# TissueImageAnalytics/cerberus

Measured on AMD Instinct MI355X. Metric: Mpx/sec WSI tiled inference (all heads), higher is better.
Workload: dtype f32

## Files before the change

### cerberus_amd/csrc/cerb_api.hip

```cpp
#include "cerb_net.h"

static thread_local std::string g_err;
int cerb_set_error(const std::string& m) {
    g_err = m;
    return 1;
}
extern "C" int cerb_version(void) { return 4; }
extern "C" const char* cerb_last_error(void) { return g_err.c_str(); }
std::atomic<long long> g_devbuf_bytes{0};
extern "C" size_t cerb_device_bytes_held(void) { const long long v = g_devbuf_bytes.load(); return v > 0 ? (size_t)v : 0; }
thread_local hipStream_t g_call_stream = nullptr;

static int alloc_dev(cerb_net* net, size_t bytes, void** out) {
    if (net->reusing) {
        if (net->reuse_cursor >= net->n_finalize_allocs || net->dev_alloc_bytes[net->reuse_cursor] != bytes)
            return fail("reload: the tensors do not have the shapes the handle was finalized with");
        *out = net->dev_allocs[net->reuse_cursor++];
        return 0;
    }
    void* d = nullptr;
    HIP_OK(hipMalloc(&d, bytes));
    net->dev_allocs.push_back(d);
    net->dev_alloc_bytes.push_back(bytes);
    *out = d;
// ... 718 lines not shown
            cur = net->x[li + 1].p;
            inpl = planes;
            continue;
        }
        for (int b = 0; b < kLayers[li]; ++b) {
            const std::string p = "backbone.layer" + std::to_string(li + 1) + "." + std::to_string(b);
            const int stride = (b == 0 && li > 0) ? 2 : 1;
            const int hin = (b == 0) ? Hi : hh, win = (b == 0) ? Wi : ww;
            float* t1 = net->ta.p;
            float* outb = ((kLayers[li] - 1 - b) % 2 == 0) ? net->x[li + 1].p : net->tb.p;
            const float* idt = cur;
            if (run_conv(net, p + ".conv1", {.in = cur, .out = t1, .N = N, .H = hin, .W = win, .relu = 1}, st)) return 1;
            if (stride != 1 || inpl != planes) {
                if (run_conv(net, p + ".downsample", {.in = cur, .out = net->pool.p, .N = N, .H = hin, .W = win}, st)) return 1;
                idt = net->pool.p;
            }
            if (run_conv(net, p + ".conv2", {.in = t1, .resid = idt, .out = outb, .N = N, .H = hh, .W = ww, .relu = 1}, st)) return 1;
            cur = outb;
            inpl = planes;
        }
    }
    if (run_conv(net, "conv_map", {.in = net->x[4].p, .out = net->cm.p, .N = N, .H = hs[4], .W = ws[4]}, st)) return 1;

    const long long tile_stride = io->tile_stride ? io->tile_stride : (long long)out_h * out_w;
    const long long row_stride = io->row_stride ? io->row_stride : out_w;
    if (net->pc_idx >= 0) {
        const bool want = io->out && io->out[net->pc_idx];
        const bool wantl = io->logits && io->logits[net->pc_idx];
        if (want || wantl) {
            PatchClassParams pp;
            memset(&pp, 0, sizeof(pp));
            pp.x4 = net->x[4].p; pp.bn1_s = net->pc_bn1s; pp.bn1_b = net->pc_bn1b; pp.w1t = net->pc_w1t; pp.b1 = net->pc_b1;
            pp.w2t = net->pc_w2t; pp.b2 = net->pc_b2;
            pp.N = N; pp.Hf = hs[4]; pp.Wf = ws[4]; pp.out_ch = net->dec[net->pc_idx].out_ch;
            pp.out_h = out_h; pp.out_w = out_w;
            pp.logits = wantl ? io->logits[net->pc_idx] : nullptr;
            pp.out = want ? (float*)io->out[net->pc_idx] : nullptr;
            pp.tile_off = io->tile_off; pp.tile_stride = tile_stride; pp.row_stride = row_stride;
            PROF("patch_class", "patch_class", 2.0 * N * (512.0 * 256 + 256.0 * pp.out_ch), HIP_OK(cerb_launch_patch_class(pp, st)));
        }
    }
    if (D) {
        const float* skips[4] = {net->x[3].p, net->x[2].p, net->x[1].p, net->x0.p};
        const float* prev = net->cm.p;
        long long prev_gs = 0;
        const int oc[4] = {128, 64, 64, 64};
        int roi_out[4][4], roi_mid[4][4], roi_sum[4][4];
        const bool any_logits = [&] {
            if (!io->logits) return false;
            for (size_t k = 0; k < net->dec.size(); ++k)
                if (io->logits[k]) return true;
            return false;
        }();
        const bool use_roi = net->crop_roi && (net->conv_algo == 1 || net->conv_algo >= 5) && !any_logits && (out_h < H || out_w < W);
        if (use_roi) {
            int y0 = (int)((H - out_h) * 0.5), x0 = (int)((W - out_w) * 0.5), y1 = y0 + out_h, x1 = x0 + out_w;
            for (int u = 3; u >= 0; --u) {
                const int hh = hs[3 - u], ww = ws[3 - u];
                auto widen = [&](int* r, const int* in, int d) {
                    r[0] = std::max(0, (in[0] - d) & ~3); r[1] = std::min(hh, (in[1] + d + 3) & ~3);
                    r[2] = std::max(0, (in[2] - d) & ~3); r[3] = std::min(ww, (in[3] + d + 3) & ~3);
                };
                const int win[4] = {y0, y1, x0, x1};
                widen(roi_out[u], win, 0);
                widen(roi_mid[u], roi_out[u], 1);
                widen(roi_sum[u], roi_mid[u], 1);
                y0 = std::max(0, roi_sum[u][0] / 2 - 1); y1 = std::min(hh / 2, (roi_sum[u][1] - 1) / 2 + 2);
                x0 = std::max(0, roi_sum[u][2] / 2 - 1); x1 = std::min(ww / 2, (roi_sum[u][3] - 1) / 2 + 2);
            }
        }
        bool feat_planar = false, prev_planar = false;
        for (int u = 0; u < 4; ++u) {
            const int hh = hs[3 - u], ww = ws[3 - u];
            const std::string n0 = "dec." + std::to_string(u) + ".0", n1 = "dec." + std::to_string(u) + ".1";
            const int cmid = net->conv[n0].cout;
            const int cin0 = net->conv[n0].cin;
            const int* r_sum = use_roi ? roi_sum[u] : nullptr;
            const int* r_mid = use_roi ? roi_mid[u] : nullptr;
            const int* r_out = use_roi ? roi_out[u] : nullptr;
            if (level_is_planar[u]) {
                PlanarBuf &bs = net->dec_sum[u], &bm = net->dec_mid[u];
                const int cout1 = net->conv[n1].cout;
                PlanarBuf& bo = cout1 == cin0 ? bs : net->dec_out[u];
                if (bs.ensure((int)D, N, hh, ww, cin0, st) || bm.ensure((int)D, N, hh, ww, cmid, st) || (&bo != &bs && bo.ensure((int)D, N, hh, ww, cout1, st)))
                    return fail_alloc();
                PROF(n0 + ".up", kPlanarEntryFamily[u], 0.0, HIP_OK(cerb_launch_upsample2_add_planar(skips[u], prev, bs.b.p, (int)D, N, hh, ww, cin0, prev_gs, bs.gs(), r_sum, prev_planar ? 1 : 0, st)));
                if (run_conv(net, n0, {.in = bs.b.p, .out = bm.b.p, .N = N, .H = hh, .W = ww, .relu = 1, .in_gs = bs.gs(), .roi = r_mid, .planar_out_gs = bm.gs(), .site = u}, st)) return 1;
                if (run_conv(net, n1, {.in = bm.b.p, .out = bo.b.p, .N = N, .H = hh, .W = ww, .relu = 1, .in_gs = bm.gs(), .roi = r_out, .planar_out_gs = bo.gs(), .site = u}, st)) return 1;
                if (u == 3) feat_planar = true;
                prev = bo.b.p;
                prev_gs = bo.gs();
                prev_planar = true;
                continue;
            }
            if (prev_planar) return fail("internal: a tile-planar decoder level feeds an NHWC one");
            if (net->conv_algo && net->conv[n0].wino) {
                PROF(n0 + ".up", "upsample2_add", 0.0, HIP_OK(cerb_launch_upsample2_add(skips[u], prev, net->dsum.p, (int)D, N, hh, ww, cin0, prev_gs, r_sum, st)));
                if (run_conv(net, n0, {.in = net->dsum.p, .out = net->dmid.p, .N = N, .H = hh, .W = ww, .relu = 1, .in_gs = (long long)N * hh * ww * cin0, .roi = r_mid}, st)) return 1;
            } else if (run_conv(net, n0, {.in = skips[u], .prev = prev, .out = net->dmid.p, .N = N, .H = hh, .W = ww, .relu = 1, .mode = 1, .prev_gs = prev_gs}, st)) return 1;
            if (run_conv(net, n1, {.in = net->dmid.p, .out = net->dout[u].p, .N = N, .H = hh, .W = ww, .relu = 1, .in_gs = (long long)N * hh * ww * cmid, .roi = r_out}, st)) return 1;
            prev = net->dout[u].p;
            prev_gs = (long long)N * hh * ww * oc[u];
        }
        HeadParams hps[8];
        int n_hp = 0;
        double head_flops = 0.0;
        for (size_t k = 0; k < net->dense_idx.size(); ++k) {
            const int di = net->dense_idx[k];
            const size_t tk = (size_t)net->trunk_of[k];
            const DecoderCfg& d = net->dec[di];
            const bool want = io->out && io->out[di];
            const bool wantl = io->logits && io->logits[di];
            if (!(want || wantl)) continue;
            HeadParams hp;
            memset(&hp, 0, sizeof(hp));
            hp.feat = feat_planar ? net->dec_sum[3].b.p + tk * net->dec_sum[3].gs() : net->dout[3].p + tk * (size_t)N * H * W * 64;
            hp.feat_planar = feat_planar ? 1 : 0;
            hp.pl_byp = cerb_planar_blocks(H);
            hp.pl_bxp = cerb_planar_blocks(W);
            hp.w1p = net->head_w1[k]; hp.b1 = net->head_b1[k]; hp.w2p = net->head_w2[k]; hp.b2 = net->head_b2[k]; hp.w2q = net->head_w2q[k];
            hp.N = N; hp.H = H; hp.W = W; hp.out_ch = d.out_ch; hp.kind = d.kind;
            hp.crop_y0 = (int)((H - out_h) * 0.5); hp.crop_x0 = (int)((W - out_w) * 0.5);
            hp.out_h = want ? out_h : 0; hp.out_w = want ? out_w : 0;
            hp.roi = use_roi ? 1 : 0;
            hp.logits = wantl ? io->logits[di] : nullptr;
            hp.absmax_bits = io->logit_absmax ? io->logit_absmax + di : nullptr;
            if (want) {
                if (d.kind == 0) hp.out_inst = (float*)io->out[di];
                else if (io->type_is_u8) hp.out_type_u8 = (unsigned char*)io->out[di];
                else hp.out_type_i64 = (long long*)io->out[di];
            }
            hp.tile_off = io->tile_off; hp.tile_stride = tile_stride; hp.row_stride = row_stride;
            const double head_px = hp.roi ? (double)out_h * (((hp.crop_x0 + out_w + 15) / 16 - hp.crop_x0 / 16) * 16.0) : (double)H * W;
            const double fl = 2.0 * N * head_px * (64.0 * 96 + 96.0 * d.out_ch);
            if (net->head_algo == 0) {
                PROF("head." + d.name, "head", fl, HIP_OK(cerb_launch_head(hp, st)));
            } else {
                if (n_hp == 8) {
                    PROF("heads", "head_group", head_flops, HIP_OK(cerb_launch_head_group(hps, n_hp, st, net->head_algo == 1 ? 1 : 0)));
                    n_hp = 0;
                    head_flops = 0.0;
                }
                hps[n_hp++] = hp;
                head_flops += fl;
            }
        }
        if (n_hp > 0) {
            PROF("heads", "head_group", head_flops, HIP_OK(cerb_launch_head_group(hps, n_hp, st, net->head_algo == 1 ? 1 : 0)));
        }
    }
    if (io->feats) {
        const float* src[6] = {net->x0.p, net->x[1].p, net->x[2].p, net->x[3].p, net->cm.p, net->x[4].p};
        const size_t nb[6] = {(size_t)N * H * W * 64, (size_t)N * hs[1] * ws[1] * 64, (size_t)N * hs[2] * ws[2] * 128,
                              (size_t)N * hs[3] * ws[3] * 256, (size_t)N * hs[4] * ws[4] * 256, (size_t)N * hs[4] * ws[4] * 512};
        for (int i = 0; i < 6; ++i)
            if (io->feats[i]) HIP_OK(hipMemcpyAsync(io->feats[i], src[i], nb[i] * 4, hipMemcpyDeviceToDevice, st));
    }
    return 0;
}

extern "C" int cerb_net_begin_reload(cerb_net* net) {
    if (!net) return fail("cerb_net_begin_reload: null handle");
    HIP_OK(hipDeviceSynchronize());
    while (net->dev_allocs.size() > net->n_finalize_allocs) {
        (void)hipFree(net->dev_allocs.back());
        net->dev_allocs.pop_back();
        net->dev_alloc_bytes.pop_back();
    }
    net->reusing = true;
    net->reuse_cursor = 0;
    net->param_slots.clear();
    net->conv.clear();
    net->bn.clear();
    net->raw.clear();
    net->grads.clear();
    net->head_w1.clear(); net->head_b1.clear(); net->head_w2.clear(); net->head_b2.clear(); net->head_w2q.clear();
    net->head_rw1.clear(); net->head_rb1.clear(); net->head_rw2.clear(); net->head_rb2.clear();
    net->host.clear();
    net->finalized = false;
    return 0;
}
// ... 176 lines not shown
```

### cerberus_amd/csrc/net_kernels.hip

```cpp
#include "cerb_common.h"

struct StemParams {
    const unsigned char* tiles;
    const float* tiles_f32;
    const float* wpack;
    const float* bias;
    float* out;
    int N, H, W, tiles_x, tiles_y;
    int relu;
};

template <bool F32IN>
__global__ __launch_bounds__(256, 2) void stem_conv7x7_kernel(StemParams p) {
    constexpr int TH = 8, TW = 32, IH = TH + 6, IW = TW + 6, ROW = 120;
    __shared__ __attribute__((aligned(16))) float wl[7 * 12 * 2 * 64];
    __shared__ __attribute__((aligned(16))) float xl[IH * ROW];
    const int tid = threadIdx.x, lane = tid & 63, wave = tid >> 6, j = lane & 31, h = lane >> 5;
    for (int i = tid; i < 7 * 12 * 2 * 64; i += 256) wl[i] = p.wpack[i];
    const int ntile = p.N * p.tiles_y * p.tiles_x;
    for (int tile = blockIdx.x; tile < ntile; tile += gridDim.x) {
        int t_ = tile;
        const int tx = t_ % p.tiles_x;
        t_ /= p.tiles_x;
        const int ty = t_ % p.tiles_y;
        const int n = t_ / p.tiles_y;
        const int oy0 = ty * TH, ox0 = tx * TW;
        __syncthreads();
        const unsigned char* img = F32IN ? nullptr : p.tiles + (long long)n * p.H * p.W * 3;
        const float* imgf = F32IN ? p.tiles_f32 + (long long)n * p.H * p.W * 3 : nullptr;
        for (int i = tid; i < IH * ROW; i += 256) {
            const int iy = i / ROW, c = i % ROW;
            const int gy = oy0 - 3 + iy, gx = ox0 - 3 + c / 3;
            float v = 0.f;
            if (c < IW * 3 && gy >= 0 && gy < p.H && gx >= 0 && gx < p.W) {
                const long long at = ((long long)gy * p.W + gx) * 3 + c % 3;
                v = (F32IN ? imgf[at] : (float)img[at]) / 255.0f;
            }
            xl[i] = v;
        }
        __syncthreads();
        f32x16 acc[2][2];
#pragma unroll
        for (int s = 0; s < 2; ++s)
#pragma unroll
            for (int q = 0; q < 2; ++q)
#pragma unroll
                for (int r = 0; r < 16; ++r) acc[s][q][r] = 0.f;
        const int b0 = (wave * 2 + 0) * ROW + j * 3 + h;
        const int b1 = (wave * 2 + 1) * ROW + j * 3 + h;
#pragma unroll
        for (int ky = 0; ky < 7; ++ky) {
#pragma unroll
            for (int t = 0; t < 12; ++t) {
                const float a0 = wl[((ky * 12 + t) * 2 + 0) * 64 + lane];
                const float a1 = wl[((ky * 12 + t) * 2 + 1) * 64 + lane];
                const float x0 = xl[b0 + ky * ROW + 2 * t];
                const float x1 = xl[b1 + ky * ROW + 2 * t];
                acc[0][0] = __builtin_amdgcn_mfma_f32_32x32x2f32(a0, x0, acc[0][0], 0, 0, 0);
                acc[1][0] = __builtin_amdgcn_mfma_f32_32x32x2f32(a1, x0, acc[1][0], 0, 0, 0);
                acc[0][1] = __builtin_amdgcn_mfma_f32_32x32x2f32(a0, x1, acc[0][1], 0, 0, 0);
                acc[1][1] = __builtin_amdgcn_mfma_f32_32x32x2f32(a1, x1, acc[1][1], 0, 0, 0);
            }
        }
#pragma unroll
        for (int q = 0; q < 2; ++q) {
            const int oy = oy0 + wave * 2 + q, ox = ox0 + j;
            if (oy >= p.H || ox >= p.W) continue;
            float* o = p.out + (((long long)n * p.H + oy) * p.W + ox) * 64;
#pragma unroll
            for (int s = 0; s < 2; ++s)
#pragma unroll
                for (int rq = 0; rq < 4; ++rq) {
                    const int co = s * 32 + rq * 8 + h * 4;
                    f32x4 v = {acc[s][q][rq * 4 + 0], acc[s][q][rq * 4 + 1], acc[s][q][rq * 4 + 2], acc[s][q][rq * 4 + 3]};
                    v = v + *reinterpret_cast<const f32x4*>(p.bias + co);
                    const float floor_ = p.relu ? 0.f : -3.402823466e38f;
                    v[0] = fmaxf(v[0], floor_);
                    v[1] = fmaxf(v[1], floor_);
                    v[2] = fmaxf(v[2], floor_);
                    v[3] = fmaxf(v[3], floor_);
                    *reinterpret_cast<f32x4*>(o + co) = v;
                }
        }
    }
}

hipError_t cerb_launch_stem(StemParams p, hipStream_t st) {
    p.tiles_x = (p.W + 31) / 32;
    p.tiles_y = (p.H + 7) / 8;
    const long long ntile = (long long)p.N * p.tiles_x * p.tiles_y;
    const unsigned grid = (unsigned)(ntile < 256 * 6 ? ntile : 256 * 6);
    if (p.tiles) hipLaunchKernelGGL(stem_conv7x7_kernel<false>, dim3(grid), dim3(256), 0, st, p);
    else hipLaunchKernelGGL(stem_conv7x7_kernel<true>, dim3(grid), dim3(256), 0, st, p);
    return hipGetLastError();
}

__global__ void maxpool3x3s2_kernel(const float* __restrict__ in, float* __restrict__ out, int N, int H, int W, int C, int Ho, int Wo) {
    const long long total = (long long)N * Ho * Wo * (C / 4);
    const long long per_xcd = gridDim.x / 8, vb = (long long)(blockIdx.x & 7) * per_xcd + (blockIdx.x >> 3);
    for (long long i = vb * (long long)blockDim.x + threadIdx.x; i < total; i += (long long)gridDim.x * blockDim.x) {
        const int c4 = (int)(i % (C / 4));
        long long r = i / (C / 4);
        const int ox = (int)(r % Wo);
        r /= Wo;
        const int oy = (int)(r % Ho);
        const int n = (int)(r / Ho);
        f32x4 m = {-INFINITY, -INFINITY, -INFINITY, -INFINITY};
#pragma unroll
        for (int ky = 0; ky < 3; ++ky) {
            const int y = oy * 2 - 1 + ky;
            if (y < 0 || y >= H) continue;
#pragma unroll
            for (int kx = 0; kx < 3; ++kx) {
                const int x = ox * 2 - 1 + kx;
                if (x < 0 || x >= W) continue;
                const f32x4 v = *reinterpret_cast<const f32x4*>(in + (((long long)n * H + y) * W + x) * C + c4 * 4);
                m[0] = fmaxf(m[0], v[0]);
                m[1] = fmaxf(m[1], v[1]);
                m[2] = fmaxf(m[2], v[2]);
                m[3] = fmaxf(m[3], v[3]);
            }
        }
        *reinterpret_cast<f32x4*>(out + i * 4) = m;
    }
}

__global__ void maxpool3x3s2_idx_kernel(const float* __restrict__ in, float* __restrict__ out, unsigned* __restrict__ idx, int N, int H, int W, int C, int Ho, int Wo) {
    const long long total = (long long)N * Ho * Wo * (C / 4);
    const long long per_xcd = gridDim.x / 8, vb = (long long)(blockIdx.x & 7) * per_xcd + (blockIdx.x >> 3);
    for (long long i = vb * (long long)blockDim.x + threadIdx.x; i < total; i += (long long)gridDim.x * blockDim.x) {
        const int c4 = (int)(i % (C / 4));
        long long r = i / (C / 4);
        const int ox = (int)(r % Wo);
        r /= Wo;
        const int oy = (int)(r % Ho);
        const int n = (int)(r / Ho);
        f32x4 m = {-INFINITY, -INFINITY, -INFINITY, -INFINITY};
        unsigned w0 = 0, w1 = 0, w2 = 0, w3 = 0;
        bool first = true;
#pragma unroll
        for (int ky = 0; ky < 3; ++ky) {
            const int y = oy * 2 - 1 + ky;
            if (y < 0 || y >= H) continue;
#pragma unroll
            for (int kx = 0; kx < 3; ++kx) {
                const int x = ox * 2 - 1 + kx;
                if (x < 0 || x >= W) continue;
                const f32x4 v = *reinterpret_cast<const f32x4*>(in + (((long long)n * H + y) * W + x) * C + c4 * 4);
                const unsigned k = (unsigned)(ky * 3 + kx);
                if (first || v[0] > m[0]) w0 = k;
                if (first || v[1] > m[1]) w1 = k;
                if (first || v[2] > m[2]) w2 = k;
                if (first || v[3] > m[3]) w3 = k;
                first = false;
                m[0] = fmaxf(m[0], v[0]);
                m[1] = fmaxf(m[1], v[1]);
                m[2] = fmaxf(m[2], v[2]);
                m[3] = fmaxf(m[3], v[3]);
            }
        }
        *reinterpret_cast<f32x4*>(out + i * 4) = m;
        idx[i] = w0 | (w1 << 8) | (w2 << 16) | (w3 << 24);
    }
}

hipError_t cerb_launch_maxpool_idx(const float* in, float* out, unsigned* idx, int N, int H, int W, int C, hipStream_t st) {
    const int Ho = (H + 2 - 3) / 2 + 1, Wo = (W + 2 - 3) / 2 + 1;
    const long long total = (long long)N * Ho * Wo * (C / 4);
    long long blocks = ((total + 255) / 256 + 7) / 8 * 8;
    if (blocks > 256 * 64) blocks = 256 * 64;
    hipLaunchKernelGGL(maxpool3x3s2_idx_kernel, dim3((unsigned)blocks), dim3(256), 0, st, in, out, idx, N, H, W, C, Ho, Wo);
    return hipGetLastError();
}

// ... 883 lines not shown
```

### cerberus_amd/csrc/cerb_net.h

```cpp
#ifndef CERB_NET_H
#define CERB_NET_H
#include <hip/hip_runtime.h>

#include <algorithm>
#include <cmath>
#include <cstdio>
#include <cstdlib>
#include <cstring>
#include <map>
#include <atomic>
#include <string>
#include <vector>

#include "../../include/cerberus_hip.h"
#include "cerb_common.h"
#include "conv_plan.h"

hipError_t cerb_launch_conv(const ConvParams& p, int ks, int stride, int mode, hipStream_t st);
hipError_t cerb_launch_wino(ConvParams p, hipStream_t st);
hipError_t cerb_launch_wino4(ConvParams p, hipStream_t st);
hipError_t cerb_launch_wino4b(ConvParams p, hipStream_t st);
int cerb_wino4b_bn_blocks(const ConvParams& p);
bool cerb_wino4b_packed(const ConvParams& p);
hipError_t cerb_launch_wino4p(ConvParams p, hipStream_t st);
hipError_t cerb_launch_upsample2_add_planar(const float* skip, const float* prev, float* out, int groups, int N, int H, int W, int C, long long prev_gs,
                                            long long out_gs, const int* roi, int prev_planar, hipStream_t st);
hipError_t cerb_launch_upsample2_add(const float* skip, const float* prev, float* out, int groups, int N, int H, int W, int C,
                                     long long prev_gs, const int* roi, hipStream_t st);
extern "C" int cerb_conv_chunk(int ks, int stride);
struct StemParams {
    const unsigned char* tiles;
    const float* tiles_f32;
    const float* wpack;
    const float* bias;
    float* out;
    int N, H, W, tiles_x, tiles_y;
    int relu;
};
hipError_t cerb_launch_stem(StemParams p, hipStream_t st);
size_t cerb_bn_workspace_bytes(int groups, long long rows, int C);
hipError_t cerb_launch_bn_stats(const float* x, long long group_stride, long long rows, int C, int groups, float eps, float* mean, float* rstd,
                                float* var_unbiased, void* ws, hipStream_t st);
hipError_t cerb_launch_bn_apply(float* x, const float* src, const float* resid, long long group_stride, long long rows, int C, int groups, const float* mean,
                                const float* rstd, const float* gamma, const float* beta, int relu, hipStream_t st);
hipError_t cerb_launch_bn_finalize(const double* partial, int blocks, long long rows, int C, float eps, float* mean, float* rstd, float* var_unbiased, hipStream_t st,
                                   int groups = 1, void* fold_ws = nullptr);
size_t cerb_bn_fold_workspace_bytes(int groups, int C);
hipError_t cerb_launch_pointwise(const float* in, const float* w, const float* bias, float* out, long long rows, int cin, int cout, const float* in_scale,
                                 hipStream_t st, double* bn_part = nullptr, int* bn_blocks = nullptr);
hipError_t cerb_launch_crop_gap(const float* x, int N, int H, int W, int C, int y0, int ch, int x0, int cw, float* out, hipStream_t st);
hipError_t cerb_launch_copy_multi(int count, float* const* dst, const float* const* src, const long long* n, void** dev_tab, size_t* dev_bytes,
                                  std::vector<char>* host_prev, hipStream_t st);
hipError_t cerb_launch_bn_bwd(const float* dz, const float* z, const float* y, float* dy, float* dresid, long long group_stride, long long rows, int C, int groups,
                              const float* mean, const float* rstd, const float* gamma, const float* beta, float* dgamma, float* dbeta, int relu, int dy_assign, void* ws, hipStream_t st, unsigned long long eval_mask = 0, int dresid_assign = 0,
                              const double* pre_part = nullptr, int pre_bpg = 0);
int cerb_head_bwd2_blocks();
hipError_t cerb_launch_conv_bwd(const float* x, const float* dy, const float* w, float* dx, float* dw, float* db, int G, int N, int H, int W, int Cin, int Cout,
                                int ks, int stride, long long x_gs, hipStream_t st);
hipError_t cerb_launch_stem_wgrad(const unsigned char* tiles, const float* dy, float* dw, int N, int H, int W, hipStream_t st);
hipError_t cerb_launch_maxpool_bwd(const float* x, const float* ypool, const float* dy, float* dx, int N, int H, int W, int C, hipStream_t st);
hipError_t cerb_launch_maxpool_idx(const float* in, float* out, unsigned* idx, int N, int H, int W, int C, hipStream_t st);
hipError_t cerb_launch_maxpool_bwd_idx(const unsigned* idx, const float* dy, float* dx, int N, int H, int W, int C, hipStream_t st);
bool cerb_upadd_bwd_fused_ok(int H, int W, int C, int G);
hipError_t cerb_launch_upadd_bwd(const float* dout, float* dskip, float* dprev, int G, int N, int H, int W, int C, long long prev_gs, int shared_prev, hipStream_t st,
                                 unsigned group_mask = 0xffffffffu, int skip_assign = 0, int prev_assign = 0);
hipError_t cerb_launch_pointwise_bwd(const float* x, const float* dy, const float* w, float* dx, float* dw, float* db, long long rows, int cin, int cout,
                                     const float* in_scale, int dx_assign, hipStream_t st);
hipError_t cerb_launch_crop_gap_bwd(const float* dg, float* dx, int N, int H, int W, int C, int y0, int ch, int x0, int cw, hipStream_t st);
hipError_t cerb_launch_adam(float* p, const float* g, float* m, float* v, long long n, float lr, float b1, float b2, float eps, int step, hipStream_t st);
size_t cerb_wgrad_workspace_bytes(int G, int N, int Ho, int Wo, int Cin, int Cout, int ks, int* slices_out);
size_t cerb_stem_wgrad_workspace_bytes();
hipError_t cerb_launch_pack_stem(const float* w_raw, float* out, hipStream_t st);
struct PackJob {
    const float* w;
    float* out;
    long long total;
    int cout, cin, kind, a, b, pad;
};
hipError_t cerb_launch_pack_multi(const PackJob* jobs, int count, void** dev_tab, size_t* dev_bytes, std::vector<char>* host_prev, hipStream_t st);
hipError_t cerb_launch_adam_multi(int count, float* const* p, const float* const* g, float* const* m, float* const* v, const long long* n, float lr, float b1,
                                  float b2, float eps, int step, hipStream_t st);
hipError_t cerb_launch_pack_conv(const float* w_raw, float* out, int cout, int cin, int ks, int chunk, hipStream_t st);
hipError_t cerb_launch_pack_wino(const float* w_raw, float* out, int cout, int cin, int dgrad, hipStream_t st);
hipError_t cerb_launch_pack_wino4(const float* w_raw, float* out, int cout, int cin, int dgrad, int chunk32, int groups, hipStream_t st);
hipError_t cerb_launch_dilate2(const float* dy, float* d, long long n, int H, int W, int C, hipStream_t st);
size_t cerb_pw_wgrad_small_workspace_bytes(long long rows, int cin, int cout);
hipError_t cerb_launch_pw_wgrad_small(const float* x, const float* dy, float* dw, long long rows, int cin, int cout, void* ws, hipStream_t st);
size_t cerb_pw_bwd_small_workspace_bytes(long long rows, int cin, int cout);
hipError_t cerb_launch_pw_bwd_small(const float* x, const float* dy, const float* w, float* dx, float* dw, float* db, long long rows, int cin, int cout,
                                    int dx_assign, void* ws, hipStream_t st);
hipError_t cerb_launch_stem_wgrad_mfma(const unsigned char* tiles, const float* dy, float* dw, int N, int H, int W, void* ws, hipStream_t st);
hipError_t cerb_launch_colsum(const float* d, long long group_stride, long long rows, int C, int G, float* out, void* ws, hipStream_t st);
bool cerb_wgrad_wino_supported(int H, int W, int Cin, int Cout);
size_t cerb_wgrad_wino_workspace_bytes(int G, int N, int H, int W, int Cin, int Cout);
hipError_t cerb_launch_wgrad_wino(const float* x, const float* dy, float* dw, int G, int N, int H, int W, int Cin, int Cout, long long x_gs, void* ws, hipStream_t st,
                                  float* db);
hipError_t cerb_launch_wgrad(const float* x, const float* dy, float* dw, int G, int N, int H, int W, int Cin, int Cout, int ks, int stride, long long x_gs, void* ws,
                             hipStream_t st, float* db = nullptr);
bool cerb_head_train_supported(long long rows, int cin, int chid, int out);
hipError_t cerb_launch_head_fwd1(const float* prev, const float* w1, const float* b1, float* hid, long long rows, double* bn_part, int* bn_blocks, hipStream_t st,
                                 const float* const* in_bn = nullptr);
hipError_t cerb_launch_head_fwd2(const float* hid, const float* mean, const float* rstd, const float* gamma, const float* beta, const float* w2, const float* b2,
                                 float* logits, long long rows, int out, hipStream_t st);
size_t cerb_head_bwd_workspace_bytes(long long rows, int out);
hipError_t cerb_launch_head_bwd1(const float* hid, const float* dlog, const float* mean, const float* rstd, const float* gamma, const float* beta, const float* w2,
                                 float* dw2, float* db2, float* dgamma, float* dbeta, long long rows, int out, void* ws, hipStream_t st);
hipError_t cerb_launch_head_bwd2(const float* hid, const float* dlog, const float* prev, const float* mean, const float* rstd, const float* gamma, const float* beta,
                                 const float* dgamma, const float* dbeta, const float* w1, const float* w2, float* dprev, float* dw1, float* db1, long long rows, int out,
                                 int eval_mode, int assign, void* ws, hipStream_t st, const float* const* in_bn = nullptr, double* in_part = nullptr);
hipError_t cerb_launch_maxpool(const float* in, float* out, int N, int H, int W, int C, hipStream_t st);
hipError_t cerb_launch_maxpool_planar(const float* in, float* out, int N, int H, int W, int C, hipStream_t st);
hipError_t cerb_launch_planar_to_nhwc(const float* in, float* out, int N, int H, int W, int C, hipStream_t st);
hipError_t cerb_launch_head(const HeadParams& p, hipStream_t st);
hipError_t cerb_launch_head_group(const HeadParams* heads, int n_heads, hipStream_t st, int w2_44);
struct PatchClassParams {
    const float* x4;
    const float* bn1_s;
    const float* bn1_b;
    const float* w1t;
    const float* b1;
    const float* w2t;
    const float* b2;
// ... 208 lines not shown
```

Measured before the change: 157.8.

## Double-buffer stem input tiles with register prefetch and trim K padding

The 7x7 stem conv now prefetches the next tile's pixels into registers (packed 4-byte loads for uint8 input) while the current tile's MFMAs run. It then converts them into a second LDS buffer, so global load latency overlaps compute. It also drops the 12th K step, which appears to multiply only zero padding, hoists bias loads out of the tile loop, and adds an env cap on stem grid size. In the decoder, the upsample-add sum is computed once and shared across heads when the previous level has no per-group stride. The cost is higher register and LDS use and a more intricate boundary-masking path.

```diff
diff --git a/cerberus_amd/csrc/cerb_api.hip b/cerberus_amd/csrc/cerb_api.hip
--- a/cerberus_amd/csrc/cerb_api.hip
+++ b/cerberus_amd/csrc/cerb_api.hip
@@ -824,10 +824,11 @@
                 PlanarBuf &bs = net->dec_sum[u], &bm = net->dec_mid[u];
                 const int cout1 = net->conv[n1].cout;
                 PlanarBuf& bo = cout1 == cin0 ? bs : net->dec_out[u];
-                if (bs.ensure((int)D, N, hh, ww, cin0, st) || bm.ensure((int)D, N, hh, ww, cmid, st) || (&bo != &bs && bo.ensure((int)D, N, hh, ww, cout1, st)))
+                const int sum_groups = prev_gs == 0 && &bo != &bs ? 1 : (int)D;
+                if (bs.ensure(sum_groups, N, hh, ww, cin0, st) || bm.ensure((int)D, N, hh, ww, cmid, st) || (&bo != &bs && bo.ensure((int)D, N, hh, ww, cout1, st)))
                     return fail_alloc();
-                PROF(n0 + ".up", kPlanarEntryFamily[u], 0.0, HIP_OK(cerb_launch_upsample2_add_planar(skips[u], prev, bs.b.p, (int)D, N, hh, ww, cin0, prev_gs, bs.gs(), r_sum, prev_planar ? 1 : 0, st)));
-                if (run_conv(net, n0, {.in = bs.b.p, .out = bm.b.p, .N = N, .H = hh, .W = ww, .relu = 1, .in_gs = bs.gs(), .roi = r_mid, .planar_out_gs = bm.gs(), .site = u}, st)) return 1;
+                PROF(n0 + ".up", kPlanarEntryFamily[u], 0.0, HIP_OK(cerb_launch_upsample2_add_planar(skips[u], prev, bs.b.p, sum_groups, N, hh, ww, cin0, prev_gs, bs.gs(), r_sum, prev_planar ? 1 : 0, st)));
+                if (run_conv(net, n0, {.in = bs.b.p, .out = bm.b.p, .N = N, .H = hh, .W = ww, .relu = 1, .in_gs = sum_groups == 1 ? 0 : bs.gs(), .roi = r_mid, .planar_out_gs = bm.gs(), .site = u}, st)) return 1;
                 if (run_conv(net, n1, {.in = bm.b.p, .out = bo.b.p, .N = N, .H = hh, .W = ww, .relu = 1, .in_gs = bm.gs(), .roi = r_out, .planar_out_gs = bo.gs(), .site = u}, st)) return 1;
                 if (u == 3) feat_planar = true;
                 prev = bo.b.p;
@@ -837,8 +838,9 @@
             }
             if (prev_planar) return fail("internal: a tile-planar decoder level feeds an NHWC one");
             if (net->conv_algo && net->conv[n0].wino) {
-                PROF(n0 + ".up", "upsample2_add", 0.0, HIP_OK(cerb_launch_upsample2_add(skips[u], prev, net->dsum.p, (int)D, N, hh, ww, cin0, prev_gs, r_sum, st)));
-                if (run_conv(net, n0, {.in = net->dsum.p, .out = net->dmid.p, .N = N, .H = hh, .W = ww, .relu = 1, .in_gs = (long long)N * hh * ww * cin0, .roi = r_mid}, st)) return 1;
+                const int sum_groups = prev_gs == 0 ? 1 : (int)D;
+                PROF(n0 + ".up", "upsample2_add", 0.0, HIP_OK(cerb_launch_upsample2_add(skips[u], prev, net->dsum.p, sum_groups, N, hh, ww, cin0, prev_gs, r_sum, st)));
+                if (run_conv(net, n0, {.in = net->dsum.p, .out = net->dmid.p, .N = N, .H = hh, .W = ww, .relu = 1, .in_gs = sum_groups == 1 ? 0 : (long long)N * hh * ww * cin0, .roi = r_mid}, st)) return 1;
             } else if (run_conv(net, n0, {.in = skips[u], .prev = prev, .out = net->dmid.p, .N = N, .H = hh, .W = ww, .relu = 1, .mode = 1, .prev_gs = prev_gs}, st)) return 1;
             if (run_conv(net, n1, {.in = net->dmid.p, .out = net->dout[u].p, .N = N, .H = hh, .W = ww, .relu = 1, .in_gs = (long long)N * hh * ww * cmid, .roi = r_out}, st)) return 1;
             prev = net->dout[u].p;
diff --git a/cerberus_amd/csrc/net_kernels.hip b/cerberus_amd/csrc/net_kernels.hip
--- a/cerberus_amd/csrc/net_kernels.hip
+++ b/cerberus_amd/csrc/net_kernels.hip
@@ -12,74 +12,124 @@
 
 template <bool F32IN>
 __global__ __launch_bounds__(256, 2) void stem_conv7x7_kernel(StemParams p) {
-    constexpr int TH = 8, TW = 32, IH = TH + 6, IW = TW + 6, ROW = 120;
-    __shared__ __attribute__((aligned(16))) float wl[7 * 12 * 2 * 64];
-    __shared__ __attribute__((aligned(16))) float xl[IH * ROW];
+    constexpr int TH = 8, TW = 32, IH = TH + 6, IW = TW + 6, ROW = 120, RB = IW * 3;
+    constexpr int DW = 30;
+    constexpr int NSLOT = ((F32IN ? IH * RB : IH * DW) + 255) / 256;
+    __shared__ __attribute__((aligned(16))) float wl[7 * 11 * 2 * 64];
+    __shared__ __attribute__((aligned(16))) float xl[2][IH * ROW];
     const int tid = threadIdx.x, lane = tid & 63, wave = tid >> 6, j = lane & 31, h = lane >> 5;
-    for (int i = tid; i < 7 * 12 * 2 * 64; i += 256) wl[i] = p.wpack[i];
+    for (int i = tid; i < 7 * 11 * 2 * 64; i += 256) wl[i] = p.wpack[i / (11 * 128) * (12 * 128) + i % (11 * 128)];
+    for (int i = tid; i < 2 * IH * (ROW - RB); i += 256) xl[i / (IH * (ROW - RB))][(i / (ROW - RB)) % IH * ROW + RB + i % (ROW - RB)] = 0.f;
     const int ntile = p.N * p.tiles_y * p.tiles_x;
-    for (int tile = blockIdx.x; tile < ntile; tile += gridDim.x) {
-        int t_ = tile;
-        const int tx = t_ % p.tiles_x;
-        t_ /= p.tiles_x;
-        const int ty = t_ % p.tiles_y;
-        const int n = t_ / p.tiles_y;
-        const int oy0 = ty * TH, ox0 = tx * TW;
+    struct Origin { int n, oy0, ox0; };
+    auto origin = [&](int tile) {
+        const int tx = tile % p.tiles_x;
+        tile /= p.tiles_x;
+        return Origin{tile / p.tiles_y, tile % p.tiles_y * TH, tx * TW};
+    };
+    auto col_lo = [&](const Origin& o) { return max(0, (3 - o.ox0) * 3); };
+    auto col_hi = [&](const Origin& o) { return min(RB, (p.W - o.ox0 + 3) * 3); };
+    unsigned r[NSLOT];
+    int cb[NSLOT];
+    auto request = [&](int tile, bool live) {
+        const Origin o = origin(tile);
+        const int c_lo = col_lo(o), c_hi = col_hi(o);
+#pragma unroll
+        for (int k = 0; k < NSLOT; ++k) {
+            const int slot = tid + 256 * k;
+            r[k] = 0u;
+            if constexpr (F32IN) {
+                const int iy = slot / RB, c = slot - iy * RB, gy = o.oy0 - 3 + iy;
+                if (live && slot < IH * RB && gy >= 0 && gy < p.H && c >= c_lo && c < c_hi)
+                    r[k] = __float_as_uint(p.tiles_f32[(((long long)o.n * p.H + gy) * p.W + o.ox0 - 3) * 3 + c]);
+            } else {
+                const int iy = slot / DW, d = slot - iy * DW, gy = o.oy0 - 3 + iy;
+                const long long at = (((long long)o.n * p.H + gy) * p.W + o.ox0 - 3) * 3;
+                const int mis = (int)(((unsigned)(unsigned long long)p.tiles + (unsigned)at) & 3u);
+                cb[k] = 4 * d - mis;
+                if (live && slot < IH * DW && gy >= 0 && gy < p.H && cb[k] + 3 >= c_lo && cb[k] < c_hi) r[k] = *reinterpret_cast<const unsigned*>(p.tiles + (at - mis + 4 * d));
+            }
+        }
+    };
+    auto convert = [&](int tile, float* x) {
+        const Origin o = origin(tile);
+        const int c_lo = col_lo(o), c_hi = col_hi(o);
+#pragma unroll
+        for (int k = 0; k < NSLOT; ++k) {
+            const int slot = tid + 256 * k;
+            if constexpr (F32IN) {
+                const int iy = slot / RB, c = slot - iy * RB;
+                if (slot < IH * RB) x[iy * ROW + c] = __uint_as_float(r[k]) / 255.0f;
+            } else {
+                const int iy = slot / DW;
+#pragma unroll
+                for (int e = 0; e < 4; ++e) {
+                    const int c = cb[k] + e;
+                    const unsigned char b = (unsigned char)(r[k] >> (8 * e));
+                    if (slot < IH * DW && c >= 0 && c < RB) x[iy * ROW + c] = c >= c_lo && c < c_hi ? (float)b / 255.0f : 0.f;
+                }
+            }
+        }
+    };
+    if ((int)blockIdx.x < ntile) {
+        request(blockIdx.x, true);
+        convert(blockIdx.x, xl[0]);
+    }
+    f32x4 bias[2][4];
+#pragma unroll
+    for (int s = 0; s < 2; ++s)
+#pragma unroll
+        for (int rq = 0; rq < 4; ++rq) bias[s][rq] = *reinterpret_cast<const f32x4*>(p.bias + s * 32 + rq * 8 + h * 4);
+    int buf = 0;
+    for (int tile = blockIdx.x; tile < ntile; tile += gridDim.x, buf ^= 1) {
+        const Origin o = origin(tile);
+        const int n = o.n, oy0 = o.oy0, ox0 = o.ox0;
+        const int next = tile + gridDim.x;
         __syncthreads();
-        const unsigned char* img = F32IN ? nullptr : p.tiles + (long long)n * p.H * p.W * 3;
-        const float* imgf = F32IN ? p.tiles_f32 + (long long)n * p.H * p.W * 3 : nullptr;
-        for (int i = tid; i < IH * ROW; i += 256) {
-            const int iy = i / ROW, c = i % ROW;
-            const int gy = oy0 - 3 + iy, gx = ox0 - 3 + c / 3;
-            float v = 0.f;
-            if (c < IW * 3 && gy >= 0 && gy < p.H && gx >= 0 && gx < p.W) {
-                const long long at = ((long long)gy * p.W + gx) * 3 + c % 3;
-                v = (F32IN ? imgf[at] : (float)img[at]) / 255.0f;
-            }
-            xl[i] = v;
-        }
-        __syncthreads();
+        request(next, next < ntile);
+        const float* x = xl[buf];
         f32x16 acc[2][2];
 #pragma unroll
         for (int s = 0; s < 2; ++s)
 #pragma unroll
             for (int q = 0; q < 2; ++q)
 #pragma unroll
-                for (int r = 0; r < 16; ++r) acc[s][q][r] = 0.f;
+                for (int r_ = 0; r_ < 16; ++r_) acc[s][q][r_] = 0.f;
         const int b0 = (wave * 2 + 0) * ROW + j * 3 + h;
         const int b1 = (wave * 2 + 1) * ROW + j * 3 + h;
 #pragma unroll
         for (int ky = 0; ky < 7; ++ky) {
 #pragma unroll
-            for (int t = 0; t < 12; ++t) {
-                const float a0 = wl[((ky * 12 + t) * 2 + 0) * 64 + lane];
-                const float a1 = wl[((ky * 12 + t) * 2 + 1) * 64 + lane];
-                const float x0 = xl[b0 + ky * ROW + 2 * t];
-                const float x1 = xl[b1 + ky * ROW + 2 * t];
+            for (int t = 0; t < 11; ++t) {
+                const float a0 = wl[((ky * 11 + t) * 2 + 0) * 64 + lane];
+                const float a1 = wl[((ky * 11 + t) * 2 + 1) * 64 + lane];
+                const float x0 = x[b0 + ky * ROW + 2 * t];
+                const float x1 = x[b1 + ky * ROW + 2 * t];
                 acc[0][0] = __builtin_amdgcn_mfma_f32_32x32x2f32(a0, x0, acc[0][0], 0, 0, 0);
                 acc[1][0] = __builtin_amdgcn_mfma_f32_32x32x2f32(a1, x0, acc[1][0], 0, 0, 0);
                 acc[0][1] = __builtin_amdgcn_mfma_f32_32x32x2f32(a0, x1, acc[0][1], 0, 0, 0);
                 acc[1][1] = __builtin_amdgcn_mfma_f32_32x32x2f32(a1, x1, acc[1][1], 0, 0, 0);
             }
         }
+        convert(next, xl[buf ^ 1]);
 #pragma unroll
         for (int q = 0; q < 2; ++q) {
             const int oy = oy0 + wave * 2 + q, ox = ox0 + j;
             if (oy >= p.H || ox >= p.W) continue;
-            float* o = p.out + (((long long)n * p.H + oy) * p.W + ox) * 64;
+            float* o_ = p.out + (((long long)n * p.H + oy) * p.W + ox) * 64;
 #pragma unroll
             for (int s = 0; s < 2; ++s)
 #pragma unroll
                 for (int rq = 0; rq < 4; ++rq) {
                     const int co = s * 32 + rq * 8 + h * 4;
                     f32x4 v = {acc[s][q][rq * 4 + 0], acc[s][q][rq * 4 + 1], acc[s][q][rq * 4 + 2], acc[s][q][rq * 4 + 3]};
-                    v = v + *reinterpret_cast<const f32x4*>(p.bias + co);
+                    v = v + bias[s][rq];
                     const float floor_ = p.relu ? 0.f : -3.402823466e38f;
                     v[0] = fmaxf(v[0], floor_);
                     v[1] = fmaxf(v[1], floor_);
                     v[2] = fmaxf(v[2], floor_);
                     v[3] = fmaxf(v[3], floor_);
-                    *reinterpret_cast<f32x4*>(o + co) = v;
+                    *reinterpret_cast<f32x4*>(o_ + co) = v;
                 }
         }
     }
@@ -89,7 +139,11 @@
     p.tiles_x = (p.W + 31) / 32;
     p.tiles_y = (p.H + 7) / 8;
     const long long ntile = (long long)p.N * p.tiles_x * p.tiles_y;
-    const unsigned grid = (unsigned)(ntile < 256 * 6 ? ntile : 256 * 6);
+    unsigned grid = (unsigned)(ntile < 256 * 6 ? ntile : 256 * 6);
+    if (const char* e = cerb_dev_getenv("CERB_STEM_MAX_WG")) {
+        const int max_wg = atoi(e);
+        if (max_wg > 0 && grid > (unsigned)max_wg) grid = (unsigned)max_wg;
+    }
     if (p.tiles) hipLaunchKernelGGL(stem_conv7x7_kernel<false>, dim3(grid), dim3(256), 0, st, p);
     else hipLaunchKernelGGL(stem_conv7x7_kernel<true>, dim3(grid), dim3(256), 0, st, p);
     return hipGetLastError();
```

New measurement: 159.1, median of 6. No clear change (+0.8%).

## Pipeline stem 7x7 conv with double-buffered input prefetch and persistent contiguous tiles

Applied to the files above, without the earlier changes.

Rewrites the stem 7x7 convolution kernel as a persistent kernel. Each block handles a contiguous range of tiles and uses two LDS input buffers, so the global loads for the next tile are issued into registers before the MFMA loop and written to LDS afterwards. Weights load as vector f32x4, bias is held in registers, the tap loop is trimmed to 11 taps, and the grid is sized to twice the CU count. This hides input-load latency behind compute and removes per-tile address recomputation, at the cost of more LDS and registers per block and possible occupancy pressure.

```diff
diff --git a/cerberus_amd/csrc/cerb_net.h b/cerberus_amd/csrc/cerb_net.h
--- a/cerberus_amd/csrc/cerb_net.h
+++ b/cerberus_amd/csrc/cerb_net.h
@@ -38,6 +38,7 @@
     int relu;
 };
 hipError_t cerb_launch_stem(StemParams p, hipStream_t st);
+int cerb_stem_grid(long long ntile);
 size_t cerb_bn_workspace_bytes(int groups, long long rows, int C);
 hipError_t cerb_launch_bn_stats(const float* x, long long group_stride, long long rows, int C, int groups, float eps, float* mean, float* rstd,
                                 float* var_unbiased, void* ws, hipStream_t st);
diff --git a/cerberus_amd/csrc/net_kernels.hip b/cerberus_amd/csrc/net_kernels.hip
--- a/cerberus_amd/csrc/net_kernels.hip
+++ b/cerberus_amd/csrc/net_kernels.hip
@@ -1,4 +1,6 @@
 #include "cerb_common.h"
+
+#include <type_traits>
 
 struct StemParams {
     const unsigned char* tiles;
@@ -10,8 +12,177 @@
     int relu;
 };
 
+#ifndef STEM_NT
+#define STEM_NT 11
+#endif
+#ifndef STEM_PERSIST
+#define STEM_PERSIST 1
+#endif
+#ifndef STEM_AHEAD
+#define STEM_AHEAD 1
+#endif
+#ifndef STEM_EPI
+#define STEM_EPI 1
+#endif
+#ifndef STEM_XCD
+#define STEM_XCD 0
+#endif
 template <bool F32IN>
 __global__ __launch_bounds__(256, 2) void stem_conv7x7_kernel(StemParams p) {
+    constexpr int TH = 8, TW = 32, IH = TH + 6, IW = TW + 6, ROW = 120;
+    constexpr int RB = IW * 3, NE = (IH * RB + 255) / 256;
+    constexpr int NBUF = STEM_AHEAD ? 2 : 1;
+    __shared__ __attribute__((aligned(16))) float wl[7 * 12 * 2 * 64];
+    __shared__ __attribute__((aligned(16))) float xl[NBUF * IH * ROW];
+    const int tid = threadIdx.x, lane = tid & 63, wave = tid >> 6, j = lane & 31, h = lane >> 5;
+    {
+        constexpr int NW4 = 7 * 12 * 2 * 16;
+        const f32x4* wg = reinterpret_cast<const f32x4*>(p.wpack);
+        f32x4 w4[NW4 / 256 + 1];
+#pragma unroll
+        for (int k = 0; k <= NW4 / 256; ++k) w4[k] = wg[min(tid + 256 * k, NW4 - 1)];
+#pragma unroll
+        for (int k = 0; k <= NW4 / 256; ++k) reinterpret_cast<f32x4*>(wl)[min(tid + 256 * k, NW4 - 1)] = w4[k];
+    }
+    if (tid < NBUF * IH * (ROW - RB)) xl[tid / (ROW - RB) * ROW + RB + tid % (ROW - RB)] = 0.f;
+
+    const int ntile = p.N * p.tiles_y * p.tiles_x;
+    const int lb = STEM_XCD ? xcd_remap(blockIdx.x, gridDim.x) : (int)blockIdx.x;
+    const int share = ntile / (int)gridDim.x, extra = ntile % (int)gridDim.x;
+    const int first = lb * share + min(lb, extra), count = share + (lb < extra ? 1 : 0);
+    int tx = first % p.tiles_x, ty = first / p.tiles_x % p.tiles_y, n = first / p.tiles_x / p.tiles_y;
+
+    int el_row[NE], el_px[NE], el_lds[NE], el_off[NE];
+#pragma unroll
+    for (int e = 0; e < NE; ++e) {
+        const int i = tid + 256 * e, iy = i / RB, c = i % RB;
+        const bool real = i < IH * RB;
+        el_row[e] = real ? iy : (1 << 24);
+        el_px[e] = c / 3;
+        el_lds[e] = real ? iy * ROW + c : RB;
+        el_off[e] = real ? iy * p.W * 3 + c : 0;
+    }
+    f32x4 bq[2][4];
+#pragma unroll
+    for (int s = 0; s < 2; ++s)
+#pragma unroll
+        for (int rq = 0; rq < 4; ++rq) bq[s][rq] = *reinterpret_cast<const f32x4*>(p.bias + s * 32 + rq * 8 + h * 4);
+    const float floor_ = p.relu ? 0.f : -3.402823466e38f;
+
+    typedef typename std::conditional<F32IN, float, unsigned char>::type raw_t;
+    const raw_t* src = F32IN ? reinterpret_cast<const raw_t*>(p.tiles_f32) : reinterpret_cast<const raw_t*>(p.tiles);
+    raw_t raw[NE];
+    unsigned inside = 0;
+    auto request = [&](int n_, int ty_, int tx_, bool live) {
+        const int gy0 = ty_ * TH - 3, gx0 = tx_ * TW - 3;
+        const long long org = (((long long)n_ * p.H + gy0) * p.W + gx0) * 3;
+        inside = 0;
+#pragma unroll
+        for (int e = 0; e < NE; ++e) {
+            const int gy = gy0 + el_row[e], gx = gx0 + el_px[e];
+            const bool ok = live && gy >= 0 && gy < p.H && gx >= 0 && gx < p.W;
+            inside |= ok ? 1u << e : 0u;
+            raw[e] = src[ok ? org + el_off[e] : 0];
+        }
+    };
+    auto commit = [&](float* dst) {
+#pragma unroll
+        for (int e = 0; e < NE; ++e) dst[el_lds[e]] = inside >> e & 1 ? (float)raw[e] / 255.0f : 0.f;
+    };
+    if (STEM_AHEAD && count > 0) {
+        request(n, ty, tx, true);
+        commit(xl);
+    }
+    __syncthreads();
+
+    for (int it = 0; it < count; ++it) {
+        const int oy0 = ty * TH, ox0 = tx * TW, n_cur = n;
+        if (++tx == p.tiles_x) {
+            tx = 0;
+            if (++ty == p.tiles_y) ty = 0, ++n;
+        }
+        const float* xb = xl + (STEM_AHEAD ? (it & 1) * IH * ROW : 0);
+        if constexpr (STEM_AHEAD) {
+            request(n, ty, tx, it + 1 < count);
+            __builtin_amdgcn_sched_barrier(0);
+        } else {
+            if (it) __syncthreads();
+            const unsigned char* img = F32IN ? nullptr : p.tiles + (long long)n_cur * p.H * p.W * 3;
+            const float* imgf = F32IN ? p.tiles_f32 + (long long)n_cur * p.H * p.W * 3 : nullptr;
+            for (int i = tid; i < IH * RB; i += 256) {
+                const int iy = i / RB, c = i % RB;
+                const int gy = oy0 - 3 + iy, gx = ox0 - 3 + c / 3;
+                float v = 0.f;
+                if (gy >= 0 && gy < p.H && gx >= 0 && gx < p.W) {
+                    const long long at = ((long long)gy * p.W + gx) * 3 + c % 3;
+                    v = (F32IN ? imgf[at] : (float)img[at]) / 255.0f;
+                }
+                xl[iy * ROW + c] = v;
+            }
+            __syncthreads();
+        }
+        f32x16 acc[2][2];
+#pragma unroll
+        for (int s = 0; s < 2; ++s)
+#pragma unroll
+            for (int q = 0; q < 2; ++q)
+#pragma unroll
+                for (int r = 0; r < 16; ++r) acc[s][q][r] = 0.f;
+        const int b0 = (wave * 2 + 0) * ROW + j * 3 + h;
+        const int b1 = (wave * 2 + 1) * ROW + j * 3 + h;
+#pragma unroll
+        for (int ky = 0; ky < 7; ++ky) {
+#pragma unroll
+            for (int t = 0; t < STEM_NT; ++t) {
+                const float a0 = wl[((ky * 12 + t) * 2 + 0) * 64 + lane];
+                const float a1 = wl[((ky * 12 + t) * 2 + 1) * 64 + lane];
+                const float x0 = xb[b0 + ky * ROW + 2 * t];
+                const float x1 = xb[b1 + ky * ROW + 2 * t];
+                acc[0][0] = __builtin_amdgcn_mfma_f32_32x32x2f32(a0, x0, acc[0][0], 0, 0, 0);
+                acc[1][0] = __builtin_amdgcn_mfma_f32_32x32x2f32(a1, x0, acc[1][0], 0, 0, 0);
+                acc[0][1] = __builtin_amdgcn_mfma_f32_32x32x2f32(a0, x1, acc[0][1], 0, 0, 0);
+                acc[1][1] = __builtin_amdgcn_mfma_f32_32x32x2f32(a1, x1, acc[1][1], 0, 0, 0);
+            }
+        }
+        if constexpr (STEM_AHEAD) commit(xl + ((it + 1) & 1) * IH * ROW);
+#pragma unroll
+        for (int q = 0; q < 2; ++q) {
+            const int oy = oy0 + wave * 2 + q, ox = ox0 + j;
+            if (oy >= p.H || ox >= p.W) continue;
+            float* o = p.out + (((long long)n_cur * p.H + oy) * p.W + ox) * 64;
+#pragma unroll
+            for (int s = 0; s < 2; ++s)
+#pragma unroll
+                for (int rq = 0; rq < 4; ++rq) {
+                    const int co = s * 32 + rq * 8 + h * 4;
+                    f32x4 v = {acc[s][q][rq * 4 + 0], acc[s][q][rq * 4 + 1], acc[s][q][rq * 4 + 2], acc[s][q][rq * 4 + 3]};
+                    v = v + (STEM_EPI ? bq[s][rq] : *reinterpret_cast<const f32x4*>(p.bias + co));
+                    v[0] = fmaxf(v[0], floor_);
+                    v[1] = fmaxf(v[1], floor_);
+                    v[2] = fmaxf(v[2], floor_);
+                    v[3] = fmaxf(v[3], floor_);
+                    *reinterpret_cast<f32x4*>(o + co) = v;
+                }
+        }
+        if constexpr (STEM_AHEAD) __syncthreads();
+    }
+}
+
+int cerb_stem_grid(long long ntile) {
+    static int cus[64];
+    int dev = 0, n = 0;
+    if (hipGetDevice(&dev) != hipSuccess || dev < 0 || dev >= 64) dev = 0;
+    if (!(n = cus[dev])) {
+        if (hipDeviceGetAttribute(&n, hipDeviceAttributeMultiprocessorCount, dev) != hipSuccess || n < 1) n = 256;
+        cus[dev] = n;
+    }
+    const long long resident = STEM_PERSIST ? 2ll * n : 256 * 6;
+    return (int)(ntile < resident ? ntile : resident);
+}
+
+#ifdef CERB_DEV_SWITCHES
+template <bool F32IN>
+__global__ __launch_bounds__(256, 2) void stem_ref_conv7x7_kernel(StemParams p) {
     constexpr int TH = 8, TW = 32, IH = TH + 6, IW = TW + 6, ROW = 120;
     __shared__ __attribute__((aligned(16))) float wl[7 * 12 * 2 * 64];
     __shared__ __attribute__((aligned(16))) float xl[IH * ROW];
@@ -84,12 +255,24 @@
         }
     }
 }
+#endif
 
 hipError_t cerb_launch_stem(StemParams p, hipStream_t st) {
     p.tiles_x = (p.W + 31) / 32;
     p.tiles_y = (p.H + 7) / 8;
     const long long ntile = (long long)p.N * p.tiles_x * p.tiles_y;
-    const unsigned grid = (unsigned)(ntile < 256 * 6 ? ntile : 256 * 6);
+#ifdef CERB_DEV_SWITCHES
+    {
+        const char* e = cerb_dev_getenv("CERB_STEM_REF");
+        if (e && e[0] != '0') {
+            const unsigned rgrid = (unsigned)(ntile < 256 * 6 ? ntile : 256 * 6);
+            if (p.tiles) hipLaunchKernelGGL(stem_ref_conv7x7_kernel<false>, dim3(rgrid), dim3(256), 0, st, p);
+            else hipLaunchKernelGGL(stem_ref_conv7x7_kernel<true>, dim3(rgrid), dim3(256), 0, st, p);
+            return hipGetLastError();
+        }
+    }
+#endif
+    const unsigned grid = (unsigned)cerb_stem_grid(ntile);
     if (p.tiles) hipLaunchKernelGGL(stem_conv7x7_kernel<false>, dim3(grid), dim3(256), 0, st, p);
     else hipLaunchKernelGGL(stem_conv7x7_kernel<true>, dim3(grid), dim3(256), 0, st, p);
     return hipGetLastError();
```

New measurement: 154.6 before, 154.8 after (median of 2 runs). About the same (+0.2%).
